# ReactiveBayes/RxInfer.jl

Measured on NVIDIA H100. Metric: gaussian_messages_per_sec_batched_lgssm_d4_T1000, higher is better.
Workload: dtype f32

## Files before the change

rxinfer.jl_b200/csrc/rxg_lgssm_cluster.cuh:

```cuda
#pragma once
#include <cooperative_groups.h>

#include "rxg_lgssm_common.cuh"
#include "rxg_lgssm_shared.cuh"

namespace rxg {

constexpr int CL_CTAS = 8;
constexpr int CL_WARPS = 8;
constexpr int CL_L = 16;

template <int D, int M>
struct ClusterTab {
    static constexpr int FK = pad4(D * D) + pad4(D * M);
    static constexpr int EG = 2 * pad4(D * D);
    static constexpr int REC = 2 * pad4(D * D);
    static constexpr int PSI_OFF = pad4(D * D);
    static_assert(Tab<D, M>::F_OFF == 0 && Tab<D, M>::K_OFF == pad4(D * D) && Tab<D, M>::E_OFF == 0 &&
                      Tab<D, M>::G_OFF == pad4(D * D),
                  "the staged prefixes are the first FK / EG floats of the gain records");

    static __host__ __device__ int spc(int T) { return ((T + CL_L - 1) / CL_L + CL_CTAS - 1) / CL_CTAS; }
    static size_t table_floats(int T) { return (size_t)(CL_CTAS * spc(T) + CL_CTAS) * REC; }
    static size_t smem_bytes(int T) {
        const size_t S = (size_t)spc(T) * CL_L;
        return 4 * (S * (M * 32 + FK + EG) + (size_t)(spc(T) + CL_CTAS) * REC + (size_t)spc(T) * D * 32 + 2 * D * 32);
    }
};

template <int D, int M>
__global__ void __launch_bounds__(256) cluster_tables_kernel(GainWs ws, float* __restrict__ tab, int T, int spc) {
    using TB = Tab<D, M>;
    using CT = ClusterTab<D, M>;
    const int nsub = CL_CTAS * spc;
    for (int j = threadIdx.x; j < nsub; j += blockDim.x) {
        const int a = j * CL_L, e = min(a + CL_L, T);
        Mat<double, D, D> Phi = identity<double, D>(), Psi = identity<double, D>();
        for (int t = a; t < e; ++t) {
            Phi = mul(load_const<double, D, D>(ws.fwd + (size_t)t * TB::FWD_REC + TB::F_OFF), Phi);
            Psi = mul(Psi, load_const<double, D, D>(ws.bwd + (size_t)t * TB::BWD_REC + TB::G_OFF));
        }
        store_f(tab + (size_t)j * CT::REC, Phi);
        store_f(tab + (size_t)j * CT::REC + CT::PSI_OFF, Psi);
    }
    __syncthreads();
    for (int r = threadIdx.x; r < CL_CTAS; r += blockDim.x) {
        Mat<double, D, D> Phi = identity<double, D>(), Psi = identity<double, D>();
        for (int j = r * spc; j < (r + 1) * spc; ++j) {
            Phi = mul(load_const<double, D, D>(tab + (size_t)j * CT::REC), Phi);
            Psi = mul(Psi, load_const<double, D, D>(tab + (size_t)j * CT::REC + CT::PSI_OFF));
        }
        store_f(tab + (size_t)(nsub + r) * CT::REC, Phi);
        store_f(tab + (size_t)(nsub + r) * CT::REC + CT::PSI_OFF, Psi);
    }
}

template <int D>
__device__ __forceinline__ void affine_step(const float* Mx, float (&v)[D], const float (&w)[D]) {
    float Mr[pad4(D * D)];
    load_smem<pad4(D * D)>(Mx, Mr);
    float n[D];
#pragma unroll
    for (int i = 0; i < D; ++i) {
        float a = w[i];
#pragma unroll
        for (int j = 0; j < D; ++j) a = __fmaf_rn(Mr[i * D + j], v[j], a);
        n[i] = a;
    }
#pragma unroll
    for (int i = 0; i < D; ++i) v[i] = n[i];
}

template <int D, int M, bool PEER>
__global__ void __launch_bounds__(32 * CL_WARPS, 2)
lgssm_cluster_sweep_kernel(const float* __restrict__ fwd_tab, const float* __restrict__ bwd_tab,
                           const float* __restrict__ cl_tab, const float* __restrict__ y, float* __restrict__ mean,
                           float* __restrict__ cov, int T, int64_t batch, int write_cov,
                           const __grid_constant__ ModelF<D, M> mdl, const __grid_constant__ PeerOut po) {
    static_assert(M >= D, "pass B stores mu_f[t] over y_t");
    using TB = Tab<D, M>;
    using CT = ClusterTab<D, M>;
    namespace cg = cooperative_groups;
    cg::cluster_group cluster = cg::this_cluster();
    const int r = (int)cluster.block_rank();
    const int spc = CT::spc(T);
    const int S = spc * CL_L;
    const int t0 = r * S;
    const int nt = max(0, min(S, T - t0));
    const int warp = threadIdx.x >> 5, lane = threadIdx.x & 31;
    const int64_t b = ((int64_t)blockIdx.x / CL_CTAS) * 32 + lane;

    extern __shared__ __align__(16) float smem[];
    float* s_y = smem;
    float* s_fk = s_y + (size_t)S * M * 32;
    float* s_eg = s_fk + (size_t)S * CT::FK;
    float* s_sub = s_eg + (size_t)S * CT::EG;
    float* s_slice = s_sub + (size_t)spc * CT::REC;
    float* s_car = s_slice + CL_CTAS * CT::REC;
    float* s_off = s_car + (size_t)spc * D * 32;

    {
        const int tid = threadIdx.x;
        for (int p = tid; p < nt * M * 8; p += 32 * CL_WARPS) {
            const int row = p >> 3, part = p & 7;
            cp_async16(s_y + row * 32 + part * 4, y + ((int64_t)t0 * M + row) * batch + (b - lane) + part * 4);
        }
        for (int p = tid; p < nt * (CT::FK / 4); p += 32 * CL_WARPS) {
            const int s = p / (CT::FK / 4), part = p % (CT::FK / 4);
            cp_async16(s_fk + s * CT::FK + part * 4, fwd_tab + (size_t)(t0 + s) * TB::FWD_REC + part * 4);
        }
        for (int p = tid; p < nt * (CT::EG / 4); p += 32 * CL_WARPS) {
            const int s = p / (CT::EG / 4), part = p % (CT::EG / 4);
            cp_async16(s_eg + s * CT::EG + part * 4, bwd_tab + (size_t)(t0 + s) * TB::BWD_REC + part * 4);
        }
        for (int p = tid; p < spc * (CT::REC / 4); p += 32 * CL_WARPS)
            cp_async16(s_sub + p * 4, cl_tab + (size_t)r * spc * CT::REC + p * 4);
        for (int p = tid; p < CL_CTAS * (CT::REC / 4); p += 32 * CL_WARPS)
            cp_async16(s_slice + p * 4, cl_tab + (size_t)CL_CTAS * spc * CT::REC + p * 4);
        cp_async_commit();
        cp_async_wait<0>();
    }
    __syncthreads();

    auto car = [&](int j, int i) -> float& { return s_car[((size_t)j * D + i) * 32 + lane]; };
    auto off = [&](float* base, int dir, int i) -> float& { return base[(dir * D + i) * 32 + lane]; };

    for (int j = warp; j < spc; j += CL_WARPS) {
        float x[D];
#pragma unroll
        for (int i = 0; i < D; ++i) x[i] = 0.f;
#pragma unroll
        for (int q = 0; q < CL_L; ++q) {
            const int s = j * CL_L + q;
            if (s < nt) {
                float Ft[pad4(D * D)], Kt[pad4(D * M)];
                load_smem<pad4(D * D)>(s_fk + s * CT::FK, Ft);
                load_smem<pad4(D * M)>(s_fk + s * CT::FK + pad4(D * D), Kt);
                float nx[D];
#pragma unroll
                for (int i = 0; i < D; ++i) {
                    float a = Ft[i * D] * x[0];
#pragma unroll
                    for (int jj = 1; jj < D; ++jj) a = __fmaf_rn(Ft[i * D + jj], x[jj], a);
#pragma unroll
                    for (int k = 0; k < M; ++k) a = __fmaf_rn(Kt[i * M + k], s_y[(s * M + k) * 32 + lane], a);
                    nx[i] = a;
                }
#pragma unroll
                for (int i = 0; i < D; ++i) x[i] = nx[i];
            }
        }
#pragma unroll
        for (int i = 0; i < D; ++i) car(j, i) = x[i];
    }
    __syncthreads();

    if (warp == 0) {
        float z[D];
#pragma unroll
        for (int i = 0; i < D; ++i) z[i] = 0.f;
        for (int j = 0; j < spc; ++j) {
            float c[D];
#pragma unroll
            for (int i = 0; i < D; ++i) c[i] = car(j, i);
            affine_step<D>(s_sub + j * CT::REC, z, c);
        }
#pragma unroll
        for (int i = 0; i < D; ++i) off(s_off, 0, i) = z[i];
    }
    cluster.sync();
    if (warp == 0) {
        float x[D];
#pragma unroll
        for (int i = 0; i < D; ++i) x[i] = mdl.m0[i];
        for (int q = 0; q < r; ++q) {
            float* rem = cluster.map_shared_rank(s_off, q);
            float c[D];
#pragma unroll
            for (int i = 0; i < D; ++i) c[i] = off(rem, 0, i);
            affine_step<D>(s_slice + q * CT::REC, x, c);
        }
        for (int j = 0; j < spc; ++j) {
            float c[D];
#pragma unroll
            for (int i = 0; i < D; ++i) { c[i] = car(j, i); car(j, i) = x[i]; }
            affine_step<D>(s_sub + j * CT::REC, x, c);
        }
    }
    __syncthreads();

    for (int j = warp; j < spc; j += CL_WARPS) {
        float x[D];
#pragma unroll
        for (int i = 0; i < D; ++i) x[i] = car(j, i);
#pragma unroll
        for (int q = 0; q < CL_L; ++q) {
            const int s = j * CL_L + q;
            if (s < nt) {
                float Ft[pad4(D * D)], Kt[pad4(D * M)], yt[M];
                load_smem<pad4(D * D)>(s_fk + s * CT::FK, Ft);
                load_smem<pad4(D * M)>(s_fk + s * CT::FK + pad4(D * D), Kt);
#pragma unroll
                for (int k = 0; k < M; ++k) yt[k] = s_y[(s * M + k) * 32 + lane];
                float nx[D];
#pragma unroll
                for (int i = 0; i < D; ++i) {
                    float a = Ft[i * D] * x[0];
#pragma unroll
                    for (int jj = 1; jj < D; ++jj) a = __fmaf_rn(Ft[i * D + jj], x[jj], a);
#pragma unroll
                    for (int k = 0; k < M; ++k) a = __fmaf_rn(Kt[i * M + k], yt[k], a);
                    nx[i] = a;
                }
#pragma unroll
                for (int i = 0; i < D; ++i) { x[i] = nx[i]; s_y[(s * M + i) * 32 + lane] = nx[i]; }
            }
        }
        float v[D];
#pragma unroll
        for (int i = 0; i < D; ++i) v[i] = 0.f;
#pragma unroll
        for (int q = CL_L - 1; q >= 0; --q) {
            const int s = j * CL_L + q;
            if (s < nt) {
                float Et[pad4(D * D)], Gt[pad4(D * D)];
                load_smem<pad4(D * D)>(s_eg + s * CT::EG, Et);
                load_smem<pad4(D * D)>(s_eg + s * CT::EG + pad4(D * D), Gt);
                float nv[D];
#pragma unroll
                for (int i = 0; i < D; ++i) {
                    float a = Et[i * D] * s_y[(s * M) * 32 + lane];
#pragma unroll
                    for (int jj = 1; jj < D; ++jj) a = __fmaf_rn(Et[i * D + jj], s_y[(s * M + jj) * 32 + lane], a);
#pragma unroll
                    for (int jj = 0; jj < D; ++jj) a = __fmaf_rn(Gt[i * D + jj], v[jj], a);
                    nv[i] = a;
                }
#pragma unroll
                for (int i = 0; i < D; ++i) v[i] = nv[i];
            }
        }
#pragma unroll
        for (int i = 0; i < D; ++i) car(j, i) = v[i];
    }
    __syncthreads();

    if (warp == 0) {
        float z[D];
#pragma unroll
        for (int i = 0; i < D; ++i) z[i] = 0.f;
        for (int j = spc - 1; j >= 0; --j) {
            float c[D];
#pragma unroll
            for (int i = 0; i < D; ++i) c[i] = car(j, i);
            affine_step<D>(s_sub + j * CT::REC + CT::PSI_OFF, z, c);
        }
#pragma unroll
        for (int i = 0; i < D; ++i) off(s_off, 1, i) = z[i];
    }
    cluster.sync();
    if (warp == 0) {
        float v[D];
#pragma unroll
        for (int i = 0; i < D; ++i) v[i] = 0.f;
        for (int q = CL_CTAS - 1; q > r; --q) {
            float* rem = cluster.map_shared_rank(s_off, q);
            float c[D];
#pragma unroll
            for (int i = 0; i < D; ++i) c[i] = off(rem, 1, i);
            affine_step<D>(s_slice + q * CT::REC + CT::PSI_OFF, v, c);
        }
        for (int j = spc - 1; j >= 0; --j) {
            float c[D];
#pragma unroll
            for (int i = 0; i < D; ++i) { c[i] = car(j, i); car(j, i) = v[i]; }
            affine_step<D>(s_sub + j * CT::REC + CT::PSI_OFF, v, c);
        }
    }
    asm volatile("barrier.cluster.arrive.release.aligned;\n" ::: "memory");
    __syncthreads();

    for (int j = warp; j < spc; j += CL_WARPS) {
        float v[D][1];
#pragma unroll
        for (int i = 0; i < D; ++i) v[i][0] = car(j, i);
#pragma unroll
        for (int q = CL_L - 1; q >= 0; --q) {
            const int s = j * CL_L + q;
            if (s < nt) {
                const int t = t0 + s;
                float Et[pad4(D * D)], Gt[pad4(D * D)];
                load_smem<pad4(D * D)>(s_eg + s * CT::EG, Et);
                load_smem<pad4(D * D)>(s_eg + s * CT::EG + pad4(D * D), Gt);
                float nv[D];
#pragma unroll
                for (int i = 0; i < D; ++i) {
                    float a = Et[i * D] * s_y[(s * M) * 32 + lane];
#pragma unroll
                    for (int jj = 1; jj < D; ++jj) a = __fmaf_rn(Et[i * D + jj], s_y[(s * M + jj) * 32 + lane], a);
#pragma unroll
                    for (int jj = 0; jj < D; ++jj) a = __fmaf_rn(Gt[i * D + jj], v[jj][0], a);
                    nv[i] = a;
                }
#pragma unroll
                for (int i = 0; i < D; ++i) {
                    v[i][0] = nv[i];
                    __stcs(mean + ((int64_t)t * D + i) * batch + b, nv[i]);
                }
                float Sst[pad4(D * D)];
                if (write_cov) {
                    load_uniform<pad4(D * D)>(bwd_tab + (size_t)t * TB::BWD_REC + TB::SS_OFF, Sst);
#pragma unroll
                    for (int i = 0; i < D * D; ++i) __stcs(cov + ((int64_t)t * D * D + i) * batch + b, Sst[i]);
                }
                if (PEER) peer_store<D, 1>(po, write_cov, t, batch, b, v, Sst);
            }
        }
    }
    asm volatile("barrier.cluster.wait.acquire.aligned;\n" ::: "memory");
}

}
```

Measured before the change: 144.2 billion.

## Write batch-invariant covariances as bulk float4 stores overlapped with table prefetch

```diff
diff --git a/rxinfer.jl_b200/csrc/rxg_lgssm_cluster.cuh b/rxinfer.jl_b200/csrc/rxg_lgssm_cluster.cuh
--- a/rxinfer.jl_b200/csrc/rxg_lgssm_cluster.cuh
+++ b/rxinfer.jl_b200/csrc/rxg_lgssm_cluster.cuh
@@ -69,6 +69,34 @@
     }
 #pragma unroll
     for (int i = 0; i < D; ++i) v[i] = n[i];
+}
+
+template <int D, int M>
+__device__ __forceinline__ void store_cov_span(const float* __restrict__ bwd_tab, float* __restrict__ cov, int64_t batch,
+                                               int T) {
+    using TB = Tab<D, M>;
+    constexpr int NT = 32 * CL_WARPS;
+    const int n4 = (int)(batch / 4);
+    const int span = D * D * T;
+    const int64_t base = (int64_t)blockIdx.x * span;
+    float4* out = reinterpret_cast<float4*>(cov) + base;
+    const int step_rows = NT / n4, step_cols = NT % n4;
+    int i = (int)threadIdx.x;
+    const int64_t q = base + i;
+    int row = (int)(q / n4), col = (int)(q - (int64_t)row * n4);
+    int cur = -1;
+    float4 v = {};
+    for (; i < span; i += NT) {
+        if (row != cur) {
+            cur = row;
+            const float s = bwd_tab[(size_t)(row / (D * D)) * TB::BWD_REC + TB::SS_OFF + row % (D * D)];
+            v = make_float4(s, s, s, s);
+        }
+        __stcs(out + i, v);
+        row += step_rows;
+        col += step_cols;
+        if (col >= n4) { col -= n4; ++row; }
+    }
 }
 
 template <int D, int M, bool PEER>
@@ -118,6 +146,7 @@
         for (int p = tid; p < CL_CTAS * (CT::REC / 4); p += 32 * CL_WARPS)
             cp_async16(s_slice + p * 4, cl_tab + (size_t)CL_CTAS * spc * CT::REC + p * 4);
         cp_async_commit();
+        if (!PEER && write_cov) store_cov_span<D, M>(bwd_tab, cov, batch, T);
         cp_async_wait<0>();
     }
     __syncthreads();
@@ -307,13 +336,15 @@
                     v[i][0] = nv[i];
                     __stcs(mean + ((int64_t)t * D + i) * batch + b, nv[i]);
                 }
-                float Sst[pad4(D * D)];
-                if (write_cov) {
-                    load_uniform<pad4(D * D)>(bwd_tab + (size_t)t * TB::BWD_REC + TB::SS_OFF, Sst);
-#pragma unroll
-                    for (int i = 0; i < D * D; ++i) __stcs(cov + ((int64_t)t * D * D + i) * batch + b, Sst[i]);
-                }
-                if (PEER) peer_store<D, 1>(po, write_cov, t, batch, b, v, Sst);
+                if constexpr (PEER) {
+                    float Sst[pad4(D * D)];
+                    if (write_cov) {
+                        load_uniform<pad4(D * D)>(bwd_tab + (size_t)t * TB::BWD_REC + TB::SS_OFF, Sst);
+#pragma unroll
+                        for (int i = 0; i < D * D; ++i) __stcs(cov + ((int64_t)t * D * D + i) * batch + b, Sst[i]);
+                    }
+                    peer_store<D, 1>(po, write_cov, t, batch, b, v, Sst);
+                }
             }
         }
     }
```

Result: faster. 149.9 billion, median of 6 (+4.0%).
